# synsin0/StreamingFlow

Hardware: AMD Instinct MI355X
Metric: ODE-steps/s on 200x200x64 BEV (GRU-ODE future-state path, full FuturePredictionODE.forward) (higher is better)
Workload: dtype f32; 1 GPU; BASELINE config 2: C=64, BEV 200x200 (latent 50x50), timeset 'shipped' (8 observations, 7 targets), variable-step euler: 10 ODE steps + 8 jumps per sample, 32 sample(s) per forward per GPU; batch_per_gpu=32, parallelism=replicas x1 (sample sharding; no data-path collective)

## Files before the change

### streamingflow_amd/csrc/conv_wino.hip

```cpp
#include "sf_math.h"
#include "sf_launch.h"

#include <cstdlib>
#include <type_traits>

namespace sf {

#ifdef SF_STAMP
static __device__ unsigned long long* g_sf_stamps = nullptr;
hipError_t set_stamp_buffer_wino(unsigned long long* p) { return hipMemcpyToSymbol(HIP_SYMBOL(g_sf_stamps), &p, sizeof(p)); }
#else
hipError_t set_stamp_buffer_wino(unsigned long long*) { return hipErrorNotSupported; }
#endif

constexpr int WN_THREADS = 512;
constexpr long SF_WINO_SPLIT_WGS_DEFAULT = 512;
typedef __attribute__((address_space(3))) void wn_lds_void;

__device__ __forceinline__ f32x4 wn_lds_read128(const float* p) {
  typedef const __attribute__((address_space(3))) f32x4 lds_f4;
  return *(lds_f4*)p;
}
__device__ __forceinline__ void wn_barrier() {
  asm volatile("" ::: "memory");
  __builtin_amdgcn_s_barrier();
  asm volatile("" ::: "memory");
}
__device__ __forceinline__ void wn_wait(const int n) {
  switch (n) {
    case 0: asm volatile("s_waitcnt vmcnt(0)" ::: "memory"); break;
    case 1: asm volatile("s_waitcnt vmcnt(1)" ::: "memory"); break;
    case 2: asm volatile("s_waitcnt vmcnt(2)" ::: "memory"); break;
    case 3: asm volatile("s_waitcnt vmcnt(3)" ::: "memory"); break;
    case 4: asm volatile("s_waitcnt vmcnt(4)" ::: "memory"); break;
    case 5: asm volatile("s_waitcnt vmcnt(5)" ::: "memory"); break;
    case 6: asm volatile("s_waitcnt vmcnt(6)" ::: "memory"); break;
    case 7: asm volatile("s_waitcnt vmcnt(7)" ::: "memory"); break;
    case 8: asm volatile("s_waitcnt vmcnt(8)" ::: "memory"); break;
    default: asm volatile("s_waitcnt vmcnt(9)" ::: "memory"); break;
  }
}

typedef float f32x2 __attribute__((ext_vector_type(2)));
__device__ __forceinline__ f32x2 wn_lo(const f32x4 v) { return (f32x2){v[0], v[1]}; }
__device__ __forceinline__ f32x2 wn_hi(const f32x4 v) { return (f32x2){v[2], v[3]}; }

template <class PT> __device__ inline int nkc_stamp(const PT& P) { return P.cin_pad >> 4; }
struct WnAxis {
  int d, r, tb, ts, nt;
  __host__ __device__ WnAxis(int N, int dil) : d(dil) {
    const int q = N / dil;
    r = N - q * dil; tb = (q + 2) >> 1; ts = (q + 1) >> 1; nt = r * tb + (dil - r) * ts;
  }
  __host__ __device__ int tiles(int p) const { return p < r ? tb : ts; }
  __host__ __device__ void decode(int X, int& p, int& t) const {
    const int nb = r * tb;
    if (X < nb) { p = X / tb; t = X - p * tb; }
    else { const int x2 = X - nb; const int pp = x2 / ts; p = r + pp; t = x2 - pp * ts; }
  }
  __host__ __device__ bool patch_coord(int pc, int p0, int t0, int n_blk, int N, int& coord) const {
    int c = 0, ph = p0, tstart = t0, left = n_blk;
    for (int run = 0; run < 4 && left > 0; ++run) {
      const int have = tiles(ph) - tstart;
      const int n = have < left ? have : left;
      if (pc < c + 2 * n + 2) {
        const int xs = 2 * tstart - 1 + (pc - c);
        coord = ph + d * xs;
        return ph < d && xs >= 0 && coord < N;
      }
      c += 2 * n + 2; left -= n; ph += 1; tstart = 0;
    }
    return false;
  }
};


__device__ __forceinline__ f32x2 wn5_sub2(const f32x2 a, const f32x2 b) {
  f32x2 r;
  asm("v_pk_add_f32 %0, %1, %2 neg_lo:[0,1] neg_hi:[0,1]" : "=v"(r) : "v"(a), "v"(b));
  return r;
}
__device__ __forceinline__ f32x4 wn5_sub4(const f32x4 a, const f32x4 b) {
  const f32x2 lo = wn5_sub2(wn_lo(a), wn_lo(b)), hi = wn5_sub2(wn_hi(a), wn_hi(b));
  return (f32x4){lo[0], lo[1], hi[0], hi[1]};
}
__device__ __forceinline__ f32x4 wn5_ld4(const float* p) { return *reinterpret_cast<const f32x4*>(p); }
__device__ __forceinline__ void wn5_st4(float* p, const f32x4 v) { *reinterpret_cast<f32x4*>(p) = v; }
__device__ __forceinline__ void wn5_act16(f32x4 (&y)[4], const int act) {
  switch (act) {
    case ACT_RELU:
#pragma unroll
      for (int k = 0; k < 4; ++k) y[k] = __builtin_elementwise_max(y[k], (f32x4){0.f, 0.f, 0.f, 0.f});
      break;
    case ACT_LRELU:
#pragma unroll
      for (int k = 0; k < 4; ++k)
#pragma unroll
        for (int q = 0; q < 4; ++q) y[k][q] = y[k][q] > 0.f ? y[k][q] : 0.1f * y[k][q];
      break;
    case ACT_SIGMOID:
#pragma unroll
      for (int k = 0; k < 4; ++k)
#pragma unroll
        for (int q = 0; q < 4; ++q) y[k][q] = __builtin_amdgcn_rcpf(1.f + __builtin_amdgcn_exp2f(-1.4426950408889634f * y[k][q]));
      break;
    case ACT_NONE: break;
    default:
#pragma unroll
      for (int k = 0; k < 4; ++k)
#pragma unroll
        for (int q = 0; q < 4; ++q) y[k][q] = spm_act(y[k][q], act);
  }
}
__device__ __forceinline__ float wn_row16_sum(float v) {
#if defined(__HIP_DEVICE_COMPILE__)
  v += __builtin_bit_cast(float, __builtin_amdgcn_update_dpp(0, __builtin_bit_cast(int, v), 0xB1, 0xF, 0xF, true));
  v += __builtin_bit_cast(float, __builtin_amdgcn_update_dpp(0, __builtin_bit_cast(int, v), 0x4E, 0xF, 0xF, true));
  v += __builtin_bit_cast(float, __builtin_amdgcn_update_dpp(0, __builtin_bit_cast(int, v), 0x141, 0xF, 0xF, true));
  v += __builtin_bit_cast(float, __builtin_amdgcn_update_dpp(0, __builtin_bit_cast(int, v), 0x140, 0xF, 0xF, true));
#endif
  return v;
}
__device__ __forceinline__ float wn_gelu(float v) { return 0.5f * v * (1.f + spm_erf(v * 0.70710678118654752440f)); }

template <bool DIL, bool CAT, int TH_ = 4>
struct Wino5Geo {
  static_assert(!(DIL && CAT), "one run structure at a time");
  static_assert(TH_ == 4 || (TH_ == 2 && !DIL), "tile rows per block");
  static constexpr int COUT_T = 64, TH = TH_, TW = 8, WT = TH * TW, NB = WT / 16;
  static constexpr int RY = 2, RX = 4;
  static constexpr int PH = 2 * TH + (DIL ? 2 * RY : 2), PW = 2 * TW + (DIL ? 2 * RX : (CAT ? 4 : 2));
  static constexpr int NPX = PH * PW;
  static constexpr int ND = (NPX * 4 + 63) / 64;
  static constexpr int NP = (ND + 7) / 8;
  static constexpr int P_FLOATS = ND * 256;
  static constexpr int V_FLOATS = 16 * WT * 16;
  static constexpr int NVB = DIL ? 1 : 2, NPB = DIL ? 2 : 1;
  static constexpr int PARK = DIL ? 512 + 64 : 0;
  static constexpr int SB = 2 * COUT_T, SC = DIL ? 0 : (CAT ? 512 : 256);
  static constexpr int T_FLOATS = 4 * 2 * WT * COUT_T;
  static_assert(NVB * V_FLOATS + NPB * P_FLOATS >= T_FLOATS, "the exchange lives over V and the patch");
  static constexpr int PV = TH_ == 2 ? 2 * 512 : 0;
  static constexpr int LDS_FLOATS = NVB * V_FLOATS + NPB * P_FLOATS + PARK + SB + SC + PV;
  static_assert((TH_ == 2 ? 3 : 2) * LDS_FLOATS * 4 <= 160 * 1024, "two workgroups per CU (three of the 16-tile form)");
};

#if !defined(SF_W5_ABL)
#define SF_W5_ABL 0
#endif
#if !defined(SF_W5_MAGIC)
#define SF_W5_MAGIC 1
#endif
template <int EPI, bool DIL = false, bool CAT = false, int TH_ = 4, int GRP = 1>
__global__ __launch_bounds__(WN_THREADS, TH_ == 2 ? 6 : 4) void conv_wino5_kernel(const ConvLaunch L) {
  static_assert(GRP == 1 || (GRP == 9 && !DIL && TH_ == 4), "tap groups: the 7x7 form");
  static_assert((EPI == EPI_LNG) == (GRP == 9), "the LayerNorm epilogue belongs to the 7x7 form");
  static_assert(EPI != EPI_SAMPLE || (!DIL && TH_ == 4), "the sampling layer: plain / concatenated 32-tile forms");
  typedef Wino5Geo<DIL, CAT, TH_> G;
  constexpr int NB = G::NB;
  constexpr int COUT_T = G::COUT_T, TH = G::TH, TW = G::TW, WT = G::WT, PW = G::PW, NP = G::NP;
  constexpr bool MODE_A = G::NVB == 2;
  extern __shared__ __attribute__((aligned(16))) float smem[];
  float* const Vbuf = smem;
  float* const Pbuf = Vbuf + G::NVB * G::V_FLOATS;
  float* const Park = Pbuf + G::NPB * G::P_FLOATS;
  float* const SBuf = Park + G::PARK;
  float* const SCbuf = SBuf + G::SB;
  float* const PVbuf = SCbuf + G::SC;
  (void)PVbuf;
  int lin_ = (int)blockIdx.x;
  const int pi_ = (int)__umulhi((unsigned)lin_, L.wn_m[0]);
  lin_ -= pi_ * L.wg_base[1];
  const ConvProblem& P = L.p[0];
  const ConvProblem& PX = L.p[pi_];
  const int tid = threadIdx.x, lane = tid & 63;
  const int wave = __builtin_amdgcn_readfirstlane(tid >> 6);
  const int H = P.Hout, W = P.Wout;
  const WnAxis ax(DIL ? W : 2, DIL ? P.dil : 1), ay(DIL ? H : 2, DIL ? P.dil : 1);
  const int tiles_x = DIL ? ax.nt : (W + 1) >> 1;
  const int tpi = tiles_x;
  const int nbx = ((CAT ? P.n_img * tiles_x : tiles_x) + TW - 1) / TW, nby = (L.wn_nty + TH - 1) / TH;
  const int ncb = P.cout_pad / COUT_T;
  const int nblk = nbx * nby * (CAT ? 1 : P.n_img), per_xcd = (nblk + 7) >> 3;
  const int lin = lin_, xcd = lin & 7, slot_ = lin >> 3;
#if SF_W5_MAGIC
  auto mdiv = [](const int nn, const unsigned m) { return m ? (int)__umulhi((unsigned)nn, m) : nn; };
  const unsigned m_ncb = L.wn_m[1], m_nbx = L.wn_m[2], m_nby = L.wn_m[3], m_tpi = L.wn_m[4];
  (void)m_tpi;
  const int tb_ = mdiv(slot_, m_ncb);
  int b = xcd * per_xcd + tb_;
  if (b >= nblk) return;
  const int bq_ = mdiv(b, m_nbx);
  const int bx = b - bq_ * nbx; b = bq_;
  const int bi_ = mdiv(b, m_nby);
  const int by = b - bi_ * nby;
  const int img = CAT ? mdiv(bx * TW, m_tpi) : bi_;
#else
  const int tb_ = slot_ / ncb;
  int b = xcd * per_xcd + tb_;
  if (b >= nblk) return;
  const int bx = b % nbx; b /= nbx;
  const int by = b % nby;
  const int img = CAT ? (bx * TW) / tpi : b / nby;
#endif
  const int ct0 = CAT ? bx * TW - img * tpi : 0;
  const int cn0 = CAT ? (tpi - ct0 < TW ? tpi - ct0 : TW) : TW;
  const int ty0 = L.wn_ty0 + by * TH, tx0 = CAT ? ct0 : bx * TW;
  int px0 = 0, pt0 = 0, py0 = 0, qt0 = 0;
  if constexpr (DIL) { ax.decode(tx0, px0, pt0); ay.decode(ty0, py0, qt0); }
  SF_STAMP_AT(L, 0);
#ifdef SF_STAMP
  SF_STAMP_VAL(L, 8, (unsigned long long)__builtin_amdgcn_s_getreg((31 << 11) | 4));
  SF_STAMP_VAL(L, 9, (unsigned long long)__builtin_amdgcn_s_getreg((31 << 11) | 20));
  SF_STAMP_VAL(L, 10, (unsigned long long)nkc_stamp(P));
#endif
  const int cout0 = (slot_ - tb_ * ncb) * COUT_T;
  const int nkc_g = P.cin_pad >> 4;
  const int nkc = GRP * nkc_g;
  const int NS = nkc * 4;
  const int c0 = P.c0;
  const int img_px_i = P.Hin * P.Win;
  const int up = DIL ? 0 : P.in_up;
  const int Win = P.Win;
#if defined(__HIP_DEVICE_COMPILE__)
  auto make_rsrc = [](const float* base, size_t bytes) {
    const unsigned nrec = bytes < 0x7fffffffull ? (unsigned)bytes : 0x7fffffffu;
    return __builtin_amdgcn_make_buffer_rsrc(const_cast<float*>(base), (short)0, (int)nrec, 0x00020000);
  };
  const size_t img_px = (size_t)P.Hin * P.Win;
  const size_t n_in = (CAT && img + 1 < P.n_img) ? 2 : 1;
  const __amdgpu_buffer_rsrc_t rsrc0 = make_rsrc(PX.in0 + (size_t)img * img_px * P.in0_cs, n_in * img_px * P.in0_cs * sizeof(float));
  const __amdgpu_buffer_rsrc_t rsrc1 = make_rsrc(PX.in1 ? PX.in1 + (size_t)img * img_px * P.in1_cs : PX.in0, PX.in1 ? n_in * img_px * P.in1_cs * sizeof(float) : 0);
  const __amdgpu_buffer_rsrc_t rsrc_u = make_rsrc(PX.w_wino, (size_t)nkc * 16 * P.cout_pad * 16 * sizeof(float));
#endif
  constexpr bool SCALED = G::SC > 0 && (EPI == EPI_AFFINE || EPI == EPI_SAMPLE);
  const bool scaled = SCALED && PX.in_scale != nullptr;
  typedef __attribute__((address_space(3))) int lds_int;
  float* const TabF = Park + 512;
  auto tab = [&](const int i) -> int { return *(const lds_int*)(TabF + i); };
  if constexpr (DIL) {
    if (tid < 72) {
      int v = 0;
      if (tid < PW) { int ix; v = ax.patch_coord(tid, px0, pt0, TW, W, ix) ? ix : -1; }
      else if (tid >= 32 && tid < 32 + G::PH) { int iy; v = ay.patch_coord(tid - 32, py0, qt0, TH, H, iy) ? iy : -1; }
      else if (tid >= 48 && tid < 60) {
        const bool isx = tid < 56;
        const int t = isx ? tx0 + (tid - 48) : ty0 + (tid - 56);
        const WnAxis& a = isx ? ax : ay;
        int pp, tt;
        a.decode(t, pp, tt);
        v = (t < a.nt && pp < P.dil) ? pp + P.dil * 2 * tt : (isx ? W : H);
      } else if (tid >= 60) {
        const bool isx = tid < 68;
        const int t = isx ? tx0 + (tid - 60) : ty0 + (tid - 68);
        int pp, tt;
        (isx ? ax : ay).decode(t, pp, tt);
        const int r = pp - (isx ? px0 : py0), lim = isx ? G::RX : G::RY;
        v = r < lim ? r : lim - 1;
      }
      *(lds_int*)(TabF + tid) = v;
    }
    asm volatile("s_waitcnt lgkmcnt(0)" ::: "memory");
    wn_barrier();
  }
  SF_STAMP_AT(L, 14);
  int pv0[NP], pv1[DIL ? 1 : NP];
  int piy[GRP > 1 ? NP : 1], pix_[GRP > 1 ? NP : 1];
  int pvs0[GRP > 1 ? NP : 1], pvs1[GRP > 1 ? NP : 1];
  (void)piy; (void)pix_; (void)pvs0; (void)pvs1;
  const int npw = G::ND / 8 + (wave < G::ND % 8 ? 1 : 0);
#pragma unroll
  for (int d = 0; d < NP; ++d) {
    const int e = (d * 8 + wave) * 64 + lane;
    const int pix = e >> 2, quad = e & 3;
    const int py = pix / PW, px = pix - py * PW;
    int iy = 2 * ty0 - 1 + py, ix = 2 * tx0 - 1 + px;
    int run = 0;
    if constexpr (CAT) {
      run = px >= 2 * cn0 + 2 ? 1 : 0;
      ix = run ? px - (2 * cn0 + 2) - 1 : ix;
    }
    bool ok = pix < G::NPX && (unsigned)iy < (unsigned)H && (unsigned)ix < (unsigned)W && (!CAT || (img + run < P.n_img && (run == 0 || cn0 < TW)));
    if constexpr (DIL) {
      const int pyc = py < G::PH ? py : 0;
      ix = tab(px); iy = tab(32 + pyc);
      ok = pix < G::NPX && ix >= 0 && iy >= 0;
    }
    const int pofs = DIL ? iy * W + ix : (iy >> up) * Win + (ix >> up) + (CAT ? run * img_px_i : 0);
    if constexpr (GRP > 1) {
      const bool in_blk = pix < G::NPX && (!CAT || (img + run < P.n_img && (run == 0 || cn0 < TW)));
      piy[d] = in_blk ? iy : -(1 << 20);
      pix_[d] = ix;
      pv0[d] = (pofs * P.in0_cs + quad * 4) * 4;
      pv1[d] = (pofs * P.in1_cs + quad * 4) * 4;
    } else {
      pv0[d] = ok ? (pofs * P.in0_cs + quad * 4) * 4 : (int)0x80000000;
      if constexpr (!DIL) pv1[d] = ok ? (pofs * P.in1_cs + quad * 4) * 4 : (int)0x80000000;
    }
  }
  int g_kc = 0, g_grp = 0;
  constexpr bool CAT_SC = CAT && G::PV == 0 && G::SC > 0;
  int run_bits = 0;
  if constexpr (CAT_SC) {
#pragma unroll
    for (int d = 0; d < NP; ++d) {
      const int pix = ((d * 8 + wave) * 64 + lane) >> 2;
      run_bits |= ((pix - (pix / PW) * PW) >= 2 * cn0 + 2 ? 1 : 0) << d;
    }
  }
  (void)run_bits;
  (void)g_kc; (void)g_grp;
  SF_STAMP_AT(L, 15);
  if constexpr (G::PV > 0) {
    static_assert(G::PV == 0 || NP == 1, "one piece per wave");
    *(lds_int*)(PVbuf + tid) = pv0[0];
    *(lds_int*)(PVbuf + 512 + tid) = pv1[0];
    asm volatile("s_waitcnt lgkmcnt(0)" ::: "memory");
  }
  auto issue_patch = [&](const int kc) {
    float* const dst = Pbuf + (G::NPB == 2 ? (kc & 1) : 0) * G::P_FLOATS;
    const bool from1 = !DIL && kc * 16 >= c0;
#if defined(__HIP_DEVICE_COMPILE__)
    if constexpr (GRP > 1) {
      if (g_kc == 0) {
        const int ga = (g_grp * 11) >> 5, gb = g_grp - 3 * ga;
        const int sy = 3 * ga - 3, sx = 3 * gb - 3;
        const int dlt = (sy * Win + sx) * 4;
#pragma unroll
        for (int d = 0; d < NP; ++d) {
          const bool okg = (unsigned)(piy[d] + sy) < (unsigned)H && (unsigned)(pix_[d] + sx) < (unsigned)W;
          pvs0[d] = okg ? pv0[d] + dlt * P.in0_cs : (int)0x80000000;
          pvs1[d] = okg ? pv1[d] + dlt * P.in1_cs : (int)0x80000000;
        }
      }
      const bool f1 = g_kc * 16 >= c0;
      const int so = f1 ? (g_kc * 16 - c0) * 4 : g_kc * 64;
#pragma unroll
      for (int d = 0; d < NP; ++d) {
        if (d >= npw) continue;
        float* const dB = dst + (d * 8 + wave) * 256;
        if (f1) {
          asm volatile("; patch from in1");
          __builtin_amdgcn_raw_ptr_buffer_load_lds(rsrc1, (wn_lds_void*)dB, 16, pvs1[d], so, 0, 0);
        } else {
          asm volatile("; patch from in0");
          __builtin_amdgcn_raw_ptr_buffer_load_lds(rsrc0, (wn_lds_void*)dB, 16, pvs0[d], so, 0, 0);
        }
      }
      if (++g_kc == nkc_g) { g_kc = 0; ++g_grp; }
      (void)kc; (void)from1;
      return;
    }
    if constexpr (G::PV > 0) {
      if (npw > 0) {
        int pv;
        asm volatile("ds_read_b32 %0, %1\n\ts_waitcnt lgkmcnt(0)" : "=v"(pv) : "v"((int)(size_t)(lds_int*)(PVbuf + (from1 ? 512 : 0) + tid)) : "memory");
        float* const dB = dst + wave * 256;
        if (from1) __builtin_amdgcn_raw_ptr_buffer_load_lds(rsrc1, (wn_lds_void*)dB, 16, pv, (kc * 16 - c0) * 4, 0, 0);
        else __builtin_amdgcn_raw_ptr_buffer_load_lds(rsrc0, (wn_lds_void*)dB, 16, pv, kc * 64, 0, 0);
      }
      return;
    }
#pragma unroll
    for (int d = 0; d < NP; ++d) {
      if (d >= npw) continue;
      float* const dB = dst + (d * 8 + wave) * 256;
      if constexpr (DIL) {
        __builtin_amdgcn_raw_ptr_buffer_load_lds(rsrc0, (wn_lds_void*)dB, 16, pv0[d], kc * 64, 0, 0);
      } else {
        if (from1) {
          asm volatile("; patch from in1");
          __builtin_amdgcn_raw_ptr_buffer_load_lds(rsrc1, (wn_lds_void*)dB, 16, pv1[d], (kc * 16 - c0) * 4, 0, 0);
        } else {
          asm volatile("; patch from in0");
          __builtin_amdgcn_raw_ptr_buffer_load_lds(rsrc0, (wn_lds_void*)dB, 16, pv0[d], kc * 64, 0, 0);
        }
      }
    }
#else
    (void)dst; (void)from1;
#endif
  };
  auto scale_patch = [&](const int kc) {
    if constexpr (SCALED) {
      if (scaled && kc * 16 < c0) {
        const f32x4 s4 = wn_lds_read128(SCbuf + kc * 16 + (lane & 3) * 4);
        f32x4 s4n = s4;
        if constexpr (CAT_SC) s4n = wn_lds_read128(SCbuf + c0 + kc * 16 + (lane & 3) * 4);
        typedef __attribute__((address_space(3))) f32x4 lds_f4w;
#pragma unroll
        for (int d = 0; d < NP; ++d) {
          if (d >= npw) continue;
          float* const q = Pbuf + ((d * 8 + wave) * 64 + lane) * 4;
          *(lds_f4w*)q = wn_lds_read128(q) * ((CAT_SC && ((run_bits >> d) & 1)) ? s4n : s4);
        }
      }
    }
  };
  const int ih = wave >> 1, hh = wave & 1;
  const int j = lane & 15, g = lane >> 4;
  const int u_voff = ((cout0 + hh * 32 + j) * 16 + g * 4) * 4;
  const int u_pos_bytes = P.cout_pad * 64;
  (void)NS; (void)u_voff; (void)u_pos_bytes;
  auto load_A = [&](const int s, const int mb) -> f32x4 {
#if defined(__HIP_DEVICE_COMPILE__)
    const int sc = s < NS ? s : NS - 1;
    const int so = (((sc >> 2) * 16 + ih * 4 + (sc & 3)) * u_pos_bytes);
    return __builtin_bit_cast(f32x4, __builtin_amdgcn_raw_buffer_load_b128(rsrc_u, u_voff + mb * 1024, so, 0));
#else
    (void)s; (void)mb; return (f32x4){0.f, 0.f, 0.f, 0.f};
#endif
  };
  const int b_off = (ih * 4 * WT + j) * 16 + ((g ^ ((j >> 2) & 2)) << 2);
  if constexpr (DIL) {
    const int quad = tid & 3, wt = (tid >> 2) % WT;
    const int tyl = wt / TW, txl = wt - tyl * TW;
    const int rx = tab(60 + txl), ry = tab(68 + tyl);
    *(__attribute__((address_space(3))) int*)(Park + tid) = ((2 * tyl + 2 * ry) * PW + 2 * txl + 2 * rx) * 16 + quad * 4;
  }
  auto transform = [&](const int kc) {
    if constexpr (WT == 16) {
      if (hh) return;
    }
    const float* const src = Pbuf + (G::NPB == 2 ? (kc & 1) : 0) * G::P_FLOATS;
    float* const dst = Vbuf + (G::NVB == 2 ? (kc & 1) : 0) * G::V_FLOATS;
    const int quad = lane & 3, wt = (tid >> 2) & (WT - 1);
    const int tyl = wt / TW, txl = wt - tyl * TW;
    const int r1 = (ih == 0) ? 0 : (ih == 2 ? 2 : 1), r2 = (ih == 3) ? 3 : (ih == 2 ? 1 : 2);
    const float sg = (ih == 1) ? 1.f : -1.f;
    const int tp = DIL ? *(const __attribute__((address_space(3))) int*)(Park + tid)
                       : ((2 * tyl) * PW + 2 * txl + ((CAT && txl >= cn0) ? 2 : 0)) * 16 + quad * 4;
    const float* const a = src + tp + r1 * PW * 16;
    const float* const bb = src + tp + r2 * PW * 16;
    float* const o = dst + ((ih * 4) * WT + wt) * 16 + ((quad ^ ((wt >> 2) & 2)) << 2);
    typedef __attribute__((address_space(3))) f32x4 lds_f4w;
    const f32x4 w0 = wn_lds_read128(a) + sg * wn_lds_read128(bb);
    const f32x4 w2 = wn_lds_read128(a + 32) + sg * wn_lds_read128(bb + 32);
    *(lds_f4w*)(o) = wn5_sub4(w0, w2);
    const f32x4 w1 = wn_lds_read128(a + 16) + sg * wn_lds_read128(bb + 16);
    *(lds_f4w*)(o + WT * 16) = w1 + w2;
    *(lds_f4w*)(o + 2 * WT * 16) = wn5_sub4(w2, w1);
    const f32x4 w3 = wn_lds_read128(a + 48) + sg * wn_lds_read128(bb + 48);
    *(lds_f4w*)(o + 3 * WT * 16) = wn5_sub4(w1, w3);
  };
  float scv = 1.f;
  if constexpr (SCALED)
    if (scaled && tid < c0) scv = PX.in_scale[(size_t)img * c0 + tid];
    if (CAT_SC && scaled && tid >= c0 && tid < 2 * c0 && img + 1 < P.n_img) scv = PX.in_scale[(size_t)(img + 1) * c0 + (tid - c0)];
  issue_patch(0);
  f32x4 A[2][2];
  A[0][0] = load_A(0, 0); A[0][1] = load_A(0, 1);
  A[1][0] = load_A(1, 0); A[1][1] = load_A(1, 1);
  float sbv = tid < COUT_T ? 1.f : 0.f;
  if (tid < 2 * COUT_T) {
    const int co = cout0 + (tid < COUT_T ? tid : tid - COUT_T);
    if (co < P.cout) {
      if (tid < COUT_T) { if (PX.scale) sbv = PX.scale[co]; }
      else if (PX.bias) sbv = PX.bias[(P.bias_per_img ? (size_t)img * P.cout : 0) + co];
    }
  }
  SF_STAMP_AT(L, 11);
  wn_wait(4);
  if constexpr (SCALED) {
    if (scaled) {
      if (tid < G::SC) SCbuf[tid] = scv;
      asm volatile("s_waitcnt lgkmcnt(0)" ::: "memory");
      wn_barrier();
      scale_patch(0);
      asm volatile("s_waitcnt lgkmcnt(0)" ::: "memory");
    }
  }
  wn_barrier();
  SF_STAMP_AT(L, 12);
  transform(0);
  SF_STAMP_AT(L, 13);
  if (tid < 2 * COUT_T) SBuf[tid] = sbv;
  if (!MODE_A) issue_patch(1);
  asm volatile("s_waitcnt lgkmcnt(0)" ::: "memory");
  wn_barrier();
  SF_STAMP_AT(L, 1);

  f32x4 acc[4][2][NB];
  int b_cur = b_off;
  auto step = [&](const int kc, auto p_c, auto first_c) {
    constexpr int p = decltype(p_c)::value, slot = p & 1;
    constexpr bool first = decltype(first_c)::value;
    const float* const vb = Vbuf + (G::NVB == 2 ? (kc & 1) : 0) * G::V_FLOATS + p * WT * 16 + b_cur;
    f32x4 Bf[NB];
#pragma unroll
    for (int nb = 0; nb < NB; ++nb) Bf[nb] = wn_lds_read128(vb + nb * 256);
    __builtin_amdgcn_sched_barrier(0);
#pragma unroll
    for (int mb = 0; mb < 2; ++mb) {
#pragma unroll
      for (int e = 0; e < 4; ++e)
#pragma unroll
        for (int nb = 0; nb < NB; ++nb) {
          const f32x4 cin = (first && e == 0) ? (f32x4){0.f, 0.f, 0.f, 0.f} : acc[p][mb][nb];
          if (SF_W5_ABL & 16) acc[p][mb][nb] = (e == 0 && nb == 0 && mb == 0) ? cin + A[slot][mb] * Bf[nb] : cin;
          else acc[p][mb][nb] = __builtin_amdgcn_mfma_f32_16x16x4f32(A[slot][mb][e], Bf[nb][e], cin, 0, 0, 0);
        }
      __builtin_amdgcn_sched_barrier(0);
      if (!(SF_W5_ABL & 4)) A[slot][mb] = load_A(kc * 4 + p + 2, mb);
      __builtin_amdgcn_sched_barrier(0);
    }
  };
  auto chunk = [&](const int kc, auto first_c, auto more_c) {
    constexpr bool more = decltype(more_c)::value;
    if (MODE_A && more && !(SF_W5_ABL & 2)) issue_patch(kc + 1);
    step(kc, std::integral_constant<int, 0>{}, first_c);
    step(kc, std::integral_constant<int, 1>{}, first_c);
    if (MODE_A && more) {
      wn_wait(4);
      scale_patch(kc + 1);
      asm volatile("s_waitcnt lgkmcnt(0)" ::: "memory");
      if (!(SF_W5_ABL & 8)) wn_barrier();
      if (!(SF_W5_ABL & 1)) transform(kc + 1);
    }
    step(kc, std::integral_constant<int, 2>{}, first_c);
    step(kc, std::integral_constant<int, 3>{}, first_c);
    if (more) {
      if constexpr (MODE_A) {
        asm volatile("s_waitcnt lgkmcnt(0)" ::: "memory");
        if (!(SF_W5_ABL & 8)) wn_barrier();
      } else {
        wn_wait(4);
        wn_barrier();
        transform(kc + 1);
        if (kc + 2 < nkc) issue_patch(kc + 2);
        asm volatile("s_waitcnt lgkmcnt(0)" ::: "memory");
        wn_barrier();
      }
    }
  };
  chunk(0, std::true_type{}, std::true_type{});
  for (int kc = 1; kc + 1 < nkc; ++kc) chunk(kc, std::false_type{}, std::true_type{});
  if constexpr (WT == 16) {
    int t2 = tid;
// ... 83 lines not shown
    const int v = (int)(pix * (unsigned)cs_a + (unsigned)c_ld) * 4;
#pragma unroll
    for (int k = 0; k < 4; ++k) oa[k] = __builtin_bit_cast(f32x4, __builtin_amdgcn_raw_buffer_load_b128(rs, okk[k] ? v : OOB, pk_[k] * cs_a * 4, 0));
  }
  if constexpr (smp) {
    if (PX.e0) {
      const __amdgpu_buffer_rsrc_t rs = make_rsrc(PX.e0 + img_base * s_half, img_span * s_half * sizeof(float));
      const int v = (int)(pix * (unsigned)s_half + (unsigned)(s_ok ? s_ch : 0)) * 4;
#pragma unroll
      for (int k = 0; k < 4; ++k)
        ev[k] = __builtin_bit_cast(f32x2, __builtin_amdgcn_raw_buffer_load_b64(rs, (okk[k] && s_ok) ? v : OOB, pk_[k] * s_half * 4, 0));
    }
  }
  if (has_b) {
    const __amdgpu_buffer_rsrc_t rs = make_rsrc(t_b + img_base * cs_b, img_span * cs_b * sizeof(float));
    const int v = (int)(pix * (unsigned)cs_b + (unsigned)(affine ? (c_ld >= P.gate_from ? c_ld - P.gate_from : 0) : c_ld)) * 4;
#pragma unroll
    for (int k = 0; k < 4; ++k) ob[k] = __builtin_bit_cast(f32x4, __builtin_amdgcn_raw_buffer_load_b128(rs, (okk[k] && (!affine || gate_lane)) ? v : OOB, pk_[k] * cs_b * 4, 0));
  }
#endif
  f32x4 as = (f32x4){1.f, 1.f, 1.f, 1.f};
  if (affine && PX.add && PX.add_scale) as = wn5_ld4(PX.add_scale + (size_t)(img + ((CAT && run_e && img_ok) ? 1 : 0)) * P.cout + c_ld);
  asm volatile("s_waitcnt lgkmcnt(0)" ::: "memory");
  wn_barrier();
  const f32x4 sc = wn_lds_read128(SBuf + cl), bi = wn_lds_read128(SBuf + COUT_T + cl);
  const int tr = wt_e * 64 + ((cq ^ (wt_e & 15)) << 2);
  SF_STAMP_AT(L, 5);
  f32x4 y[4];
#pragma unroll
  for (int bq = 0; bq < 2; ++bq) {
    const float* const tb = Tb + bq * WT * 64 + tr;
    const f32x4 t0 = wn_lds_read128(tb), t1 = wn_lds_read128(tb + 2 * WT * 64), t2 = wn_lds_read128(tb + 4 * WT * 64), t3 = wn_lds_read128(tb + 6 * WT * 64);
    y[2 * bq] = (t0 + t1) + t2;
    y[2 * bq + 1] = wn5_sub4(t1, t2 + t3);
  }
  SF_STAMP_AT(L, 6);
  if constexpr (!lng) {
#pragma unroll
    for (int k = 0; k < 4; ++k) y[k] = __builtin_elementwise_fma(y[k], sc, bi);
  }
  f32x4 y2[4];
  if constexpr (smp) {
    wn5_act16(y, P.act);
#if defined(__HIP_DEVICE_COMPILE__)
    typedef __attribute__((__vector_size__(2 * sizeof(unsigned)))) unsigned u32x2;
    const __amdgpu_buffer_rsrc_t rs_p = make_rsrc(PX.out + img_base * s_half, img_span * s_half * sizeof(float));
    const __amdgpu_buffer_rsrc_t rs_q = make_rsrc(PX.out2 ? PX.out2 + img_base * P.cout : PX.out, PX.out2 ? img_span * P.cout * sizeof(float) : 0);
    const unsigned gp0 = (unsigned)img_base + pix;
#pragma unroll
    for (int k = 0; k < 4; ++k) {
      const bool okp = okk[k] && s_ok;
      f32x2 e = ev[k];
      if (!PX.e0) {
        const float2 d = spm_philox_normal2(P.philox, P.draw, okp ? gp0 + (unsigned)pk_[k] : 0u, (unsigned)(s_ok ? s_ch : 0));
        e = (f32x2){d.x, d.y};
      }
      const f32x2 r = {y[k][0] + e[0] * (spm_softplus(y[k][2]) + 1e-8f), y[k][1] + e[1] * (spm_softplus(y[k][3]) + 1e-8f)};
      const int vp = (int)(pix * (unsigned)s_half + (unsigned)s_ch) * 4, vq = (int)(pix * (unsigned)P.cout + (unsigned)s_ch) * 4;
      __builtin_amdgcn_raw_buffer_store_b64(__builtin_bit_cast(u32x2, r), rs_p, okp ? vp : OOB, pk_[k] * s_half * 4, 0);
      if (PX.out2) {
        __builtin_amdgcn_raw_buffer_store_b64(__builtin_bit_cast(u32x2, (f32x2){y[k][0], y[k][1]}), rs_q, okp ? vq : OOB, pk_[k] * P.cout * 4, 0);
        __builtin_amdgcn_raw_buffer_store_b64(__builtin_bit_cast(u32x2, (f32x2){y[k][2], y[k][3]}), rs_q, okp ? vq + s_half * 4 : OOB, pk_[k] * P.cout * 4, 0);
      }
    }
#endif
    SF_STAMP_AT(L, 3);
    return;
  } else if constexpr (lng) {
    if (P.mode & 1) {
      const float inv_c = 1.f / (float)P.cout;
#pragma unroll
      for (int k = 0; k < 4; ++k) {
        const float mean = wn_row16_sum((y[k][0] + y[k][1]) + (y[k][2] + y[k][3])) * inv_c;
        const f32x4 dv = y[k] - (f32x4){mean, mean, mean, mean};
        const float var = wn_row16_sum((dv[0] * dv[0] + dv[1] * dv[1]) + (dv[2] * dv[2] + dv[3] * dv[3])) * inv_c;
        const float rstd = 1.f / sqrtf(var + P.eps);
        y[k] = __builtin_elementwise_fma(dv * (f32x4){rstd, rstd, rstd, rstd}, sc, bi);
      }
    }
#pragma unroll
    for (int k = 0; k < 4; ++k)
#pragma unroll
      for (int q = 0; q < 4; ++q) y[k][q] = wn_gelu(y[k][q]);
    if (PX.add) {
#pragma unroll
      for (int k = 0; k < 4; ++k) y[k] = y[k] + oa[k];
    }
  } else if constexpr (affine) {
    const bool act_last = (P.mode & 2) != 0;
    if (!act_last) wn5_act16(y, P.act);
    if (P.clamp_from >= 0) {
#pragma unroll
      for (int k = 0; k < 4; ++k)
#pragma unroll
        for (int q = 0; q < 4; ++q)
          if (c + q >= P.clamp_from) y[k][q] = fminf(fmaxf(y[k][q], P.clamp_lo), P.clamp_hi);
    }
    if (PX.add) {
      if (PX.add_scale) {
#pragma unroll
        for (int k = 0; k < 4; ++k) y[k] = __builtin_elementwise_fma(oa[k], as, y[k]);
      } else {
#pragma unroll
        for (int k = 0; k < 4; ++k) y[k] = y[k] + oa[k];
      }
    }
    if (act_last) wn5_act16(y, P.act);
    if (PX.out2) {
#pragma unroll
      for (int k = 0; k < 4; ++k) y2[k] = ob[k] * ((f32x4){1.f, 1.f, 1.f, 1.f} - y[k]);
    }
  } else {
    wn5_act16(y, P.act);
    if (P.mode & 1) {
#pragma unroll
      for (int k = 0; k < 4; ++k) y[k] = oa[k] * (y[k] - ob[k]);
    } else {
#pragma unroll
      for (int k = 0; k < 4; ++k) y[k] = ((f32x4){1.f, 1.f, 1.f, 1.f} - oa[k]) * ob[k] + oa[k] * y[k];
    }
  }
  SF_STAMP_AT(L, 7);
  __builtin_amdgcn_sched_barrier(0);
#if defined(__HIP_DEVICE_COMPILE__)
  if (affine && !DIL && P.pool2) {
    const size_t pimg = (size_t)(H >> 1) * (W >> 1);
    const __amdgpu_buffer_rsrc_t rs = make_rsrc(PX.out + (size_t)img * pimg * P.out_cs + P.out_co,
                                                n_span * pimg * P.out_cs * sizeof(float) - (size_t)P.out_co * sizeof(float));
    const unsigned ppix = (unsigned)(ty * (W >> 1) + tx) + (run_e ? (unsigned)pimg : 0u);
    const f32x4 m = __builtin_elementwise_max(__builtin_elementwise_max(y[0], y[1]), __builtin_elementwise_max(y[2], y[3]));
    __builtin_amdgcn_raw_buffer_store_b128(__builtin_bit_cast(__attribute__((__vector_size__(4 * sizeof(unsigned)))) unsigned, m), rs,
                                           okk[0] ? (int)(ppix * (unsigned)P.out_cs + (unsigned)c_ld) * 4 : OOB, 0, 0);
  } else {
    const __amdgpu_buffer_rsrc_t rs = make_rsrc(PX.out + img_base * P.out_cs + P.out_co, img_span * P.out_cs * sizeof(float) - (size_t)P.out_co * sizeof(float));
    const int v = (int)(pix * (unsigned)P.out_cs + (unsigned)c_ld) * 4;
#pragma unroll
    for (int k = 0; k < 4; ++k)
      __builtin_amdgcn_raw_buffer_store_b128(__builtin_bit_cast(__attribute__((__vector_size__(4 * sizeof(unsigned)))) unsigned, y[k]), rs, okk[k] ? v : OOB, pk_[k] * P.out_cs * 4, 0);
  }
  if (affine && PX.out2) {
    const __amdgpu_buffer_rsrc_t rs = make_rsrc(PX.out2 + img_base * P.out2_cs, img_span * P.out2_cs * sizeof(float));
    const int v = (int)(pix * (unsigned)P.out2_cs + (unsigned)(c_ld >= P.gate_from ? c_ld - P.gate_from : 0)) * 4;
#pragma unroll
    for (int k = 0; k < 4; ++k)
      __builtin_amdgcn_raw_buffer_store_b128(__builtin_bit_cast(__attribute__((__vector_size__(4 * sizeof(unsigned)))) unsigned, y2[k]), rs, (okk[k] && gate_lane) ? v : OOB, pk_[k] * P.out2_cs * 4, 0);
  }
#endif
  SF_STAMP_AT(L, 3);
#ifdef SF_STAMP
  asm volatile("s_waitcnt vmcnt(0)" ::: "memory");
  SF_STAMP_AT(L, 4);
#endif
}

__global__ void wino_weights_kernel(const float* __restrict__ w, float* __restrict__ U, int cout_pad, int cin_pad, int ksz) {
  const long idx = (long)blockIdx.x * blockDim.x + threadIdx.x;
  const int ngrp = ksz == 7 ? 9 : 1;
  if (idx >= (long)ngrp * cout_pad * cin_pad) return;
  const int grp = (int)(idx / ((long)cout_pad * cin_pad));
  const long rem = idx - (long)grp * cout_pad * cin_pad;
  const int co = (int)(rem / cin_pad), ci = (int)(rem - (long)co * cin_pad);
  const int ga = grp / 3, gb = grp - 3 * ga;
  float g[3][3];
#pragma unroll
  for (int a = 0; a < 3; ++a)
#pragma unroll
    for (int b = 0; b < 3; ++b) {
      const int ky = ksz == 7 ? 3 * ga + a - 1 : a, kx = ksz == 7 ? 3 * gb + b - 1 : b;
      g[a][b] = (ky >= 0 && ky < ksz && kx >= 0 && kx < ksz) ? w[(size_t)co * ksz * ksz * cin_pad + (size_t)(ky * ksz + kx) * cin_pad + ci] : 0.f;
    }
  float t[4][3];
#pragma unroll
  for (int b = 0; b < 3; ++b) {
    t[0][b] = g[0][b];
    t[1][b] = 0.5f * (g[0][b] + g[1][b] + g[2][b]);
    t[2][b] = 0.5f * (g[0][b] - g[1][b] + g[2][b]);
    t[3][b] = g[2][b];
  }
  const int kc = ci >> 4, cl = ci & 15, nkc = cin_pad >> 4;
#pragma unroll
  for (int i = 0; i < 4; ++i) {
    const float u0 = t[i][0], u1 = 0.5f * (t[i][0] + t[i][1] + t[i][2]), u2 = 0.5f * (t[i][0] - t[i][1] + t[i][2]), u3 = t[i][2];
    const float uu[4] = {u0, u1, u2, u3};
#pragma unroll
    for (int jj = 0; jj < 4; ++jj) U[((((size_t)grp * nkc + kc) * 16 + i * 4 + jj) * cout_pad + co) * 16 + cl] = uu[jj];
  }
}
hipError_t launch_wino_weights(const float* w, float* U, int cout_pad, int cin_pad, int ksz, hipStream_t stream) {
  const long n = (long)(ksz == 7 ? 9 : 1) * cout_pad * cin_pad;
  hipLaunchKernelGGL(wino_weights_kernel, dim3((unsigned)((n + 255) / 256)), dim3(256), 0, stream, w, U, cout_pad, cin_pad, ksz);
  return hipGetLastError();
}

static bool wino_takes_ln7(const ConvProblem& q) {
  static const int on = [] { const char* v = std::getenv("SF_WINO_LN7"); return v ? std::atoi(v) : 1; }();
  if (!on || !q.w_wino || q.KH != 7 || q.KW != 7 || q.stride != 1 || q.dil != 1 || q.pad != 3 || q.in_up || q.gather || q.gate || q.se_sum || q.in_scale ||
      q.nsplit > 1 || q.chansum || q.acc_in || q.fuse_w || q.out_planar || q.pool2 || q.add_up || q.add_scale || q.bias_per_img || q.out2)
    return false;
  if (q.cout != 64 || q.cout_pad != 64 || (q.c0 % 16) || (q.c1 % 16) || q.c0 + q.c1 != q.cin_pad || (q.cin_pad % 32)) return false;
  if (q.Hout != q.Hin || q.Wout != q.Win || q.Hout < 16 || q.Wout < 32) return false;
  static const double min_p = [] { const char* v = std::getenv("SF_WINO_LN7_MIN_P"); return v ? std::atof(v) : 65536.0; }();
  if ((double)q.n_img * q.Hout * q.Wout < min_p) return false;
  const double img_bytes = 4.0 * q.Hin * q.Win;
  if (img_bytes * q.out_cs >= 2147483648.0 || img_bytes * q.add_cs >= 2147483648.0 || img_bytes * q.in0_cs >= 2147483648.0 ||
      img_bytes * q.in1_cs >= 2147483648.0 || 4.0 * 9 * 16 * q.cout_pad * q.cin_pad >= 2147483648.0)
    return false;
  return true;
}
bool wino_takes(const ConvProblem& q, int epi) {
  if (epi == EPI_LNG) return wino_takes_ln7(q);
  if (epi == EPI_SAMPLE) {
    static const int on = [] { const char* v = std::getenv("SF_WINO_SAMPLE"); return v ? std::atoi(v) : 1; }();
    const double img_px = (double)q.Hin * q.Win;
    if (!on || q.dil != 1 || q.in_up || q.add || q.add_scale || q.pool2 || q.add_up || q.bias_per_img || q.scale || (q.cout % 8) || (q.c1 != 0) ||
        2.0 * 4.0 * img_px * q.cout >= 2147483648.0 || (!q.e0 && !q.philox))
      return false;
    return wino_takes(q, EPI_AFFINE);
  }
  if (epi != EPI_AFFINE && epi != EPI_BLEND) return false;
  if (!q.w_wino || q.KH != 3 || q.KW != 3 || q.stride != 1 || q.dil < 1 || q.pad != q.dil || (q.in_up && q.dil != 1) || q.gather || q.gate || q.se_sum ||
      (q.in_scale && (epi != EPI_AFFINE || q.dil != 1 || q.c0 > 256)) ||
      q.nsplit > 1 || q.chansum || q.acc_in || q.fuse_w || q.out_planar || (epi == EPI_AFFINE && (q.mode & 4)))
    return false;
  if (q.pool2 && (epi != EPI_AFFINE || q.dil != 1 || q.out2 || (q.Hout & 1) || (q.Wout & 1))) return false;
  if (q.add_up && (epi != EPI_AFFINE || q.dil != 1 || !q.add || (q.Hout & 1) || (q.Wout & 1))) return false;
  if ((q.c0 % 16) || (q.c1 % 16) || q.c0 + q.c1 != q.cin_pad || (q.cout_pad % 64) || (q.cout % 4)) return false;
  if (q.Hout != (q.Hin << q.in_up) || q.Wout != (q.Win << q.in_up) || q.Hout < 16 || q.Wout < 32) return false;
  if (q.dil > 1 && (q.c1 != 0 || epi != EPI_AFFINE || q.Hout / q.dil < 5 || q.Wout / q.dil < 5)) return false;
  const double img_bytes = 4.0 * q.Hin * q.Win;
  if (img_bytes * q.out_cs >= 2147483648.0 || img_bytes * q.add_cs >= 2147483648.0 || img_bytes * q.e0_cs >= 2147483648.0 ||
      img_bytes * q.e1_cs >= 2147483648.0 || img_bytes * q.out2_cs >= 2147483648.0)
    return false;
  if (img_bytes * q.in0_cs >= 2147483648.0 || img_bytes * q.in1_cs >= 2147483648.0 || 4.0 * 16 * q.cout_pad * q.cin_pad >= 2147483648.0) return false;
  return true;
}

static bool wino_cat(const ConvProblem& q) {
  static const int on = [] { const char* v = std::getenv("SF_WINO_CAT"); return v ? std::atoi(v) : 1; }();
  const int tpi = (q.Wout + 1) / 2;
  static const int cat_scaled = [] { const char* v = std::getenv("SF_WINO_CAT_SCALED"); return v ? std::atoi(v) : 1; }();
  if (!on || q.dil != 1 || q.in_up || q.n_img < 2 || tpi < 8 || q.bias_per_img || ((q.in_scale || q.add_scale) && !cat_scaled)) return false;
  const int plain = (tpi + 7) / 8 * 8;
  if (plain * 100 < tpi * 110) {
    if (q.cout_pad < 128 || plain * 100 < tpi * 104) return false;
    const char* const v = std::getenv("SF_WINO_CAT_WIDE");
    if (v && std::atoi(v) == 0) return false;
  }
  const double img_bytes = 4.0 * q.Hin * q.Win;
  const int cs = q.in0_cs > q.in1_cs ? q.in0_cs : q.in1_cs;
  const int co = q.out_cs > q.add_cs ? q.out_cs : q.add_cs;
  const int ce = q.e0_cs > q.e1_cs ? q.e0_cs : q.e1_cs;
  const int cm = co > ce ? (co > q.out2_cs ? co : q.out2_cs) : (ce > q.out2_cs ? ce : q.out2_cs);
  return 2.0 * img_bytes * cs < 2147483648.0 && 2.0 * img_bytes * cm < 2147483648.0;
}
int wino_variant(const ConvProblem& q) {
  if (q.cout_pad % 64) return -1;
  if (q.dil > 1) return 3;
  if (wino_cat(q)) return 4;
  return 2;
}
double wino_tiles(const ConvProblem& q) {
  if (q.dil > 1) return (double)q.n_img * WnAxis(q.Hout, q.dil).nt * WnAxis(q.Wout, q.dil).nt;
  return (double)q.n_img * ((q.Hout + 1) / 2) * ((q.Wout + 1) / 2);
}
static long wino5_wgs(const ConvLaunch& L, bool cat, int rows, int th) {
  const ConvProblem& P = L.p[0];
  const int tiles_x = (P.Wout + 1) / 2;
  const long nby = (rows + th - 1) / th;
  const long blocks = cat ? nby * (((long)P.n_img * tiles_x + 7) / 8) : (long)P.n_img * nby * ((tiles_x + 7) / 8);
  return ((blocks + 7) / 8) * 8 * (P.cout_pad / 64) * L.nprob;
}
template <int EPI, bool DIL = false, bool CAT = false, int TH_ = 4, int GRP = 1>
static hipError_t launch_wino5_t(const ConvLaunch& L, hipStream_t stream, const int row0 = 0, const int rows = -1) {
  typedef Wino5Geo<DIL, CAT, TH_> G;
  auto kern = conv_wino5_kernel<EPI, DIL, CAT, TH_, GRP>;
  constexpr int lds = G::LDS_FLOATS * 4;
  static bool attr_done[64] = {};
  int dev = 0;
  if (hipGetDevice(&dev) != hipSuccess || dev < 0 || dev >= 64) return hipErrorInvalidDevice;
  if (!attr_done[dev]) {
    hipError_t e = hipFuncSetAttribute(reinterpret_cast<const void*>(kern), hipFuncAttributeMaxDynamicSharedMemorySize, lds);
    if (e != hipSuccess) return e;
    attr_done[dev] = true;
  }
  const ConvProblem& P = L.p[0];
  const int tiles_x = DIL ? WnAxis(P.Wout, P.dil).nt : (P.Wout + 1) / 2, tiles_all = DIL ? WnAxis(P.Hout, P.dil).nt : (P.Hout + 1) / 2;
  const int tiles_y = rows < 0 ? tiles_all : rows;
  if (row0 < 0 || tiles_y < 1 || row0 + tiles_y > tiles_all || (DIL && tiles_y != tiles_all) || (row0 + tiles_y < tiles_all && tiles_y % G::TH)) return hipErrorInvalidValue;
  const long blocks = CAT ? (long)((tiles_y + G::TH - 1) / G::TH) * (((long)P.n_img * tiles_x + G::TW - 1) / G::TW)
                          : (long)P.n_img * ((tiles_y + G::TH - 1) / G::TH) * ((tiles_x + G::TW - 1) / G::TW);
  const long grid1 = ((blocks + 7) / 8) * 8 * (P.cout_pad / G::COUT_T), grid = grid1 * L.nprob;
  if (grid > 0x7fffffffL) return hipErrorInvalidValue;
  ConvLaunch L2 = L;
  L2.wg_base[0] = 0;
  L2.wg_base[1] = (int)grid1;
  L2.wn_ty0 = row0; L2.wn_nty = tiles_y;
  const long nbx = ((CAT ? (long)P.n_img * tiles_x : tiles_x) + G::TW - 1) / G::TW, nby = (tiles_y + G::TH - 1) / G::TH, ncb = P.cout_pad / G::COUT_T;
  if ((grid1 / 8 + 1) * ncb >= 0x100000000L || (blocks + 8) * nbx >= 0x100000000L || (blocks + 8) * nby >= 0x100000000L ||
      (nbx * G::TW + G::TW) * tiles_x >= 0x100000000L)
    return hipErrorInvalidValue;
  if (L.nprob > 1 && grid * grid1 >= 0x100000000L) return hipErrorInvalidValue;
  L2.wn_m[0] = L.nprob > 1 ? magic(grid1) : 1u;
  L2.wn_m[1] = magic(ncb); L2.wn_m[2] = magic(nbx); L2.wn_m[3] = magic(nby); L2.wn_m[4] = magic(tiles_x);
  hipLaunchKernelGGL(kern, dim3((unsigned)grid, 1, 1), dim3(WN_THREADS), lds, stream, L2);
  return hipGetLastError();
}
bool wino_same_geometry(const ConvProblem& a, const ConvProblem& b) {
  return a.n_img == b.n_img && a.Hin == b.Hin && a.Win == b.Win && a.Hout == b.Hout && a.Wout == b.Wout && a.in_up == b.in_up && a.dil == b.dil &&
         a.c0 == b.c0 && a.c1 == b.c1 && a.cin_pad == b.cin_pad && a.cout == b.cout && a.cout_pad == b.cout_pad &&
         (a.in_scale != nullptr) == (b.in_scale != nullptr) && (a.in1 != nullptr) == (b.in1 != nullptr) && (a.add != nullptr) == (b.add != nullptr) &&
         (a.add_scale != nullptr) == (b.add_scale != nullptr) && (a.out2 != nullptr) == (b.out2 != nullptr) && (a.scale != nullptr) == (b.scale != nullptr) &&
         (a.bias != nullptr) == (b.bias != nullptr) && a.in0_cs == b.in0_cs && a.in1_cs == b.in1_cs && a.add_cs == b.add_cs && a.out_cs == b.out_cs &&
         a.out_co == b.out_co && a.out2_cs == b.out2_cs && a.e0_cs == b.e0_cs && a.e1_cs == b.e1_cs && a.act == b.act && a.mode == b.mode &&
         a.gate_from == b.gate_from && a.clamp_from == b.clamp_from && a.clamp_lo == b.clamp_lo && a.clamp_hi == b.clamp_hi &&
         a.bias_per_img == b.bias_per_img && a.pool2 == b.pool2 && a.add_up == b.add_up && wino_variant(a) == wino_variant(b);
}
hipError_t launch_conv_wino(const ConvLaunch& L, int epi, hipStream_t stream) {
  if (L.nprob < 1 || L.nprob > SF_MAX_GROUP) return hipErrorInvalidValue;
  for (int i = 0; i < L.nprob; ++i)
    if (!wino_takes(L.p[i], epi) || !wino_same_geometry(L.p[0], L.p[i])) return hipErrorInvalidValue;
  const bool affine = epi == EPI_AFFINE;
  const int var = wino_variant(L.p[0]);
  if (epi == EPI_SAMPLE) {
    if (var == 2) return launch_wino5_t<EPI_SAMPLE>(L, stream);
    if (var == 4) return launch_wino5_t<EPI_SAMPLE, false, true>(L, stream);
    return hipErrorInvalidValue;
  }
  if (epi == EPI_LNG) {
    if (var == 2) return launch_wino5_t<EPI_LNG, false, false, 4, 9>(L, stream);
    if (var == 4) return launch_wino5_t<EPI_LNG, false, true, 4, 9>(L, stream);
    return hipErrorInvalidValue;
  }
  static const long small_wgs = [] { const char* v = std::getenv("SF_WINO_SMALL_WGS"); return v ? std::atol(v) : 1000L; }();
  if (var == 3) return affine ? launch_wino5_t<EPI_AFFINE, true>(L, stream) : hipErrorInvalidValue;
  if (var != 2 && var != 4) return hipErrorInvalidValue;
  const bool cat = var == 4;
  const bool only32 = cat && L.p[0].in_scale;
  auto launch = [&](const bool small, const int row0, const int rows) -> hipError_t {
    if (cat) {
      if (small) return affine ? launch_wino5_t<EPI_AFFINE, false, true, 2>(L, stream, row0, rows) : launch_wino5_t<EPI_BLEND, false, true, 2>(L, stream, row0, rows);
      return affine ? launch_wino5_t<EPI_AFFINE, false, true>(L, stream, row0, rows) : launch_wino5_t<EPI_BLEND, false, true>(L, stream, row0, rows);
    }
    if (small) return affine ? launch_wino5_t<EPI_AFFINE, false, false, 2>(L, stream, row0, rows) : launch_wino5_t<EPI_BLEND, false, false, 2>(L, stream, row0, rows);
    return affine ? launch_wino5_t<EPI_AFFINE>(L, stream, row0, rows) : launch_wino5_t<EPI_BLEND>(L, stream, row0, rows);
  };
  const int tiles_y = (L.p[0].Hout + 1) / 2;
  const bool small = !only32 && wino5_wgs(L, cat, tiles_y, 4) < small_wgs;
  const char* const sv = std::getenv("SF_WINO_SPLIT_WGS");
  const long split_wgs = sv ? std::atol(sv) : SF_WINO_SPLIT_WGS_DEFAULT;
  const int main_rows = tiles_y & ~3, rem_rows = tiles_y - main_rows;
  if (!small && !only32 && split_wgs > 0 && rem_rows > 0 && main_rows > 0 && wino5_wgs(L, cat, rem_rows, 2) >= split_wgs) {
    const hipError_t e = launch(wino5_wgs(L, cat, main_rows, 4) < small_wgs, 0, main_rows);
    return e != hipSuccess ? e : launch(true, main_rows, rem_rows);
  }
  return launch(small, 0, -1);
}

}
```

Baseline: 2149 ODE-steps/s.

## Extend 16-tile Winograd form to 7x7 tap-group, sampling and scaled-concat convs

```diff
diff --git a/streamingflow_amd/csrc/conv_wino.hip b/streamingflow_amd/csrc/conv_wino.hip
--- a/streamingflow_amd/csrc/conv_wino.hip
+++ b/streamingflow_amd/csrc/conv_wino.hip
@@ -151,11 +151,11 @@
 #if !defined(SF_W5_MAGIC)
 #define SF_W5_MAGIC 1
 #endif
-template <int EPI, bool DIL = false, bool CAT = false, int TH_ = 4, int GRP = 1>
-__global__ __launch_bounds__(WN_THREADS, TH_ == 2 ? 6 : 4) void conv_wino5_kernel(const ConvLaunch L) {
-  static_assert(GRP == 1 || (GRP == 9 && !DIL && TH_ == 4), "tap groups: the 7x7 form");
+template <int EPI, bool DIL, bool CAT, int TH_, int GRP>
+__device__ __forceinline__ void conv_wino5_body(const ConvLaunch& L) {
+  static_assert(GRP == 1 || (GRP == 9 && !DIL), "tap groups: the 7x7 form");
   static_assert((EPI == EPI_LNG) == (GRP == 9), "the LayerNorm epilogue belongs to the 7x7 form");
-  static_assert(EPI != EPI_SAMPLE || (!DIL && TH_ == 4), "the sampling layer: plain / concatenated 32-tile forms");
+  static_assert(EPI != EPI_SAMPLE || !DIL, "the sampling layer: plain / concatenated forms");
   typedef Wino5Geo<DIL, CAT, TH_> G;
   constexpr int NB = G::NB;
   constexpr int COUT_T = G::COUT_T, TH = G::TH, TW = G::TW, WT = G::WT, PW = G::PW, NP = G::NP;
@@ -287,7 +287,9 @@
       ok = pix < G::NPX && ix >= 0 && iy >= 0;
     }
     const int pofs = DIL ? iy * W + ix : (iy >> up) * Win + (ix >> up) + (CAT ? run * img_px_i : 0);
-    if constexpr (GRP > 1) {
+    if constexpr (GRP > 1 && G::PV > 0) {
+      (void)ok; (void)pofs; (void)quad;
+    } else if constexpr (GRP > 1) {
       const bool in_blk = pix < G::NPX && (!CAT || (img + run < P.n_img && (run == 0 || cn0 < TW)));
       piy[d] = in_blk ? iy : -(1 << 20);
       pix_[d] = ix;
@@ -299,9 +301,9 @@
     }
   }
   int g_kc = 0, g_grp = 0;
-  constexpr bool CAT_SC = CAT && G::PV == 0 && G::SC > 0;
+  constexpr bool CAT_SC = CAT && G::SC > 0;
   int run_bits = 0;
-  if constexpr (CAT_SC) {
+  if constexpr (CAT_SC && G::PV == 0) {
 #pragma unroll
     for (int d = 0; d < NP; ++d) {
       const int pix = ((d * 8 + wave) * 64 + lane) >> 2;
@@ -311,7 +313,7 @@
   (void)run_bits;
   (void)g_kc; (void)g_grp;
   SF_STAMP_AT(L, 15);
-  if constexpr (G::PV > 0) {
+  if constexpr (G::PV > 0 && GRP == 1) {
     static_assert(G::PV == 0 || NP == 1, "one piece per wave");
     *(lds_int*)(PVbuf + tid) = pv0[0];
     *(lds_int*)(PVbuf + 512 + tid) = pv1[0];
@@ -321,7 +323,40 @@
     float* const dst = Pbuf + (G::NPB == 2 ? (kc & 1) : 0) * G::P_FLOATS;
     const bool from1 = !DIL && kc * 16 >= c0;
 #if defined(__HIP_DEVICE_COMPILE__)
-    if constexpr (GRP > 1) {
+    if constexpr (GRP > 1 && G::PV > 0) {
+      if (g_kc == 0) {
+        int t = wave * 64 + (int)__builtin_amdgcn_mbcnt_hi(~0u, __builtin_amdgcn_mbcnt_lo(~0u, 0u));
+        asm volatile("" : "+v"(t));
+        const int ga = (g_grp * 11) >> 5, gb = g_grp - 3 * ga;
+        const int sy = 3 * ga - 3, sx = 3 * gb - 3;
+        const int dlt = (sy * Win + sx) * 4;
+        const int pix = t >> 2, quad = t & 3;
+        const int py = pix / PW, px = pix - py * PW;
+        int iy = 2 * ty0 - 1 + py, ix = 2 * tx0 - 1 + px, run = 0;
+        unsigned in_blk = pix < G::NPX ? 1u : 0u;
+        if constexpr (CAT) {
+          run = px >= 2 * cn0 + 2 ? 1 : 0;
+          ix = run ? px - (2 * cn0 + 2) - 1 : ix;
+          const int run_ok = (img + 1 < P.n_img && cn0 < TW) ? 1 : 0;
+          in_blk &= (unsigned)((run ^ 1) | run_ok);
+        }
+        const int pofs = (iy >> up) * Win + (ix >> up) + (CAT ? run * img_px_i : 0);
+        const unsigned okg = in_blk & ((unsigned)(iy + sy) < (unsigned)H ? 1u : 0u) & ((unsigned)(ix + sx) < (unsigned)W ? 1u : 0u);
+        *(lds_int*)(PVbuf + t) = okg ? (pofs * P.in0_cs + quad * 4) * 4 + dlt * P.in0_cs : (int)0x80000000;
+        *(lds_int*)(PVbuf + 512 + t) = okg ? (pofs * P.in1_cs + quad * 4) * 4 + dlt * P.in1_cs : (int)0x80000000;
+      }
+      const bool f1 = g_kc * 16 >= c0;
+      if (npw > 0) {
+        int pv;
+        asm volatile("ds_read_b32 %0, %1\n\ts_waitcnt lgkmcnt(0)" : "=v"(pv) : "v"((int)(size_t)(lds_int*)(PVbuf + (f1 ? 512 : 0) + tid)) : "memory");
+        float* const dB = dst + wave * 256;
+        if (f1) __builtin_amdgcn_raw_ptr_buffer_load_lds(rsrc1, (wn_lds_void*)dB, 16, pv, (g_kc * 16 - c0) * 4, 0, 0);
+        else __builtin_amdgcn_raw_ptr_buffer_load_lds(rsrc0, (wn_lds_void*)dB, 16, pv, g_kc * 64, 0, 0);
+      }
+      if (++g_kc == nkc_g) { g_kc = 0; g_grp = __builtin_amdgcn_readfirstlane(g_grp + 1); }
+      (void)kc; (void)from1;
+      return;
+    } else if constexpr (GRP > 1) {
       if (g_kc == 0) {
         const int ga = (g_grp * 11) >> 5, gb = g_grp - 3 * ga;
         const int sy = 3 * ga - 3, sx = 3 * gb - 3;
@@ -383,7 +418,17 @@
   };
   auto scale_patch = [&](const int kc) {
     if constexpr (SCALED) {
-      if (scaled && kc * 16 < c0) {
+      if constexpr (CAT_SC && G::PV > 0) {
+        if (scaled && kc * 16 < c0 && npw > 0) {
+          int t = tid;
+          asm volatile("" : "+v"(t));
+          const int pix = t >> 2;
+          const bool nxt = (pix - (pix / PW) * PW) >= 2 * cn0 + 2;
+          typedef __attribute__((address_space(3))) f32x4 lds_f4w;
+          float* const q = Pbuf + t * 4;
+          *(lds_f4w*)q = wn_lds_read128(q) * wn_lds_read128(SCbuf + (nxt ? c0 : 0) + kc * 16 + (t & 3) * 4);
+        }
+      } else if (scaled && kc * 16 < c0) {
         const f32x4 s4 = wn_lds_read128(SCbuf + kc * 16 + (lane & 3) * 4);
         f32x4 s4n = s4;
         if constexpr (CAT_SC) s4n = wn_lds_read128(SCbuf + c0 + kc * 16 + (lane & 3) * 4);
@@ -773,6 +818,16 @@
   SF_STAMP_AT(L, 4);
 #endif
 }
+template <int EPI, bool DIL = false, bool CAT = false, int TH_ = 4, int GRP = 1>
+__global__ __launch_bounds__(WN_THREADS, TH_ == 2 ? 6 : 4) void conv_wino5_kernel(const ConvLaunch L) {
+  static_assert(TH_ == 4 || (GRP == 1 && EPI != EPI_SAMPLE), "the 16-tile tap groups and sampling layer: conv_wino16_kernel");
+  conv_wino5_body<EPI, DIL, CAT, TH_, GRP>(L);
+}
+template <int EPI, bool CAT, int GRP>
+__global__ __launch_bounds__(WN_THREADS, 6) void conv_wino16_kernel(const ConvLaunch L) {
+  static_assert(GRP == 9 || EPI == EPI_SAMPLE, "every other 16-tile form is conv_wino5_kernel<.., 2>");
+  conv_wino5_body<EPI, false, CAT, 2, GRP>(L);
+}
 
 __global__ void wino_weights_kernel(const float* __restrict__ w, float* __restrict__ U, int cout_pad, int cin_pad, int ksz) {
   const long idx = (long)blockIdx.x * blockDim.x + threadIdx.x;
@@ -894,7 +949,10 @@
 template <int EPI, bool DIL = false, bool CAT = false, int TH_ = 4, int GRP = 1>
 static hipError_t launch_wino5_t(const ConvLaunch& L, hipStream_t stream, const int row0 = 0, const int rows = -1) {
   typedef Wino5Geo<DIL, CAT, TH_> G;
-  auto kern = conv_wino5_kernel<EPI, DIL, CAT, TH_, GRP>;
+  auto kern = [] {
+    if constexpr (TH_ == 2 && (GRP == 9 || EPI == EPI_SAMPLE)) return conv_wino16_kernel<EPI, CAT, GRP>;
+    else return conv_wino5_kernel<EPI, DIL, CAT, TH_, GRP>;
+  }();
   constexpr int lds = G::LDS_FLOATS * 4;
   static bool attr_done[64] = {};
   int dev = 0;
@@ -942,35 +1000,29 @@
     if (!wino_takes(L.p[i], epi) || !wino_same_geometry(L.p[0], L.p[i])) return hipErrorInvalidValue;
   const bool affine = epi == EPI_AFFINE;
   const int var = wino_variant(L.p[0]);
-  if (epi == EPI_SAMPLE) {
-    if (var == 2) return launch_wino5_t<EPI_SAMPLE>(L, stream);
-    if (var == 4) return launch_wino5_t<EPI_SAMPLE, false, true>(L, stream);
-    return hipErrorInvalidValue;
-  }
-  if (epi == EPI_LNG) {
-    if (var == 2) return launch_wino5_t<EPI_LNG, false, false, 4, 9>(L, stream);
-    if (var == 4) return launch_wino5_t<EPI_LNG, false, true, 4, 9>(L, stream);
-    return hipErrorInvalidValue;
-  }
+  if (epi != EPI_AFFINE && epi != EPI_BLEND && epi != EPI_SAMPLE && epi != EPI_LNG) return hipErrorInvalidValue;
   static const long small_wgs = [] { const char* v = std::getenv("SF_WINO_SMALL_WGS"); return v ? std::atol(v) : 1000L; }();
   if (var == 3) return affine ? launch_wino5_t<EPI_AFFINE, true>(L, stream) : hipErrorInvalidValue;
   if (var != 2 && var != 4) return hipErrorInvalidValue;
   const bool cat = var == 4;
-  const bool only32 = cat && L.p[0].in_scale;
+  auto launch_epi = [&](auto epi_c, auto grp_c, const bool small, const int row0, const int rows) -> hipError_t {
+    constexpr int E = decltype(epi_c)::value, GRP = decltype(grp_c)::value;
+    if (cat) return small ? launch_wino5_t<E, false, true, 2, GRP>(L, stream, row0, rows) : launch_wino5_t<E, false, true, 4, GRP>(L, stream, row0, rows);
+    return small ? launch_wino5_t<E, false, false, 2, GRP>(L, stream, row0, rows) : launch_wino5_t<E, false, false, 4, GRP>(L, stream, row0, rows);
+  };
   auto launch = [&](const bool small, const int row0, const int rows) -> hipError_t {
-    if (cat) {
-      if (small) return affine ? launch_wino5_t<EPI_AFFINE, false, true, 2>(L, stream, row0, rows) : launch_wino5_t<EPI_BLEND, false, true, 2>(L, stream, row0, rows);
-      return affine ? launch_wino5_t<EPI_AFFINE, false, true>(L, stream, row0, rows) : launch_wino5_t<EPI_BLEND, false, true>(L, stream, row0, rows);
-    }
-    if (small) return affine ? launch_wino5_t<EPI_AFFINE, false, false, 2>(L, stream, row0, rows) : launch_wino5_t<EPI_BLEND, false, false, 2>(L, stream, row0, rows);
-    return affine ? launch_wino5_t<EPI_AFFINE>(L, stream, row0, rows) : launch_wino5_t<EPI_BLEND>(L, stream, row0, rows);
+    typedef std::integral_constant<int, 1> one;
+    if (epi == EPI_LNG) return launch_epi(std::integral_constant<int, EPI_LNG>{}, std::integral_constant<int, 9>{}, small, row0, rows);
+    if (epi == EPI_SAMPLE) return launch_epi(std::integral_constant<int, EPI_SAMPLE>{}, one{}, small, row0, rows);
+    if (affine) return launch_epi(std::integral_constant<int, EPI_AFFINE>{}, one{}, small, row0, rows);
+    return launch_epi(std::integral_constant<int, EPI_BLEND>{}, one{}, small, row0, rows);
   };
   const int tiles_y = (L.p[0].Hout + 1) / 2;
-  const bool small = !only32 && wino5_wgs(L, cat, tiles_y, 4) < small_wgs;
+  const bool small = wino5_wgs(L, cat, tiles_y, 4) < small_wgs;
   const char* const sv = std::getenv("SF_WINO_SPLIT_WGS");
   const long split_wgs = sv ? std::atol(sv) : SF_WINO_SPLIT_WGS_DEFAULT;
   const int main_rows = tiles_y & ~3, rem_rows = tiles_y - main_rows;
-  if (!small && !only32 && split_wgs > 0 && rem_rows > 0 && main_rows > 0 && wino5_wgs(L, cat, rem_rows, 2) >= split_wgs) {
+  if (!small && split_wgs > 0 && rem_rows > 0 && main_rows > 0 && wino5_wgs(L, cat, rem_rows, 2) >= split_wgs) {
     const hipError_t e = launch(wino5_wgs(L, cat, main_rows, 4) < small_wgs, 0, main_rows);
     return e != hipSuccess ? e : launch(true, main_rows, rem_rows);
   }
```

Result: no change. 2152 ODE-steps/s, median of 3 (+0.2%).
